# Rongjiehuang/FastDiff

Hardware: AMD Instinct MI355X
Metric: real-time factor (audio-sec/wall-sec), N=4 reverse steps, 80x864 mel (higher is better)
Workload: dtype f32 results; 2-piece fp16 operands (22 bit) on fp16 MFMA, fp32 accumulate; GEMM as Winograd F(2,3); exact-fp32 twin; 1 GPU; BASELINE configs[1]: LJSpeech shape, batch=8 x 80x864 mel per GPU, N=4, HIP kernels + hipGraph sampler; batch_per_gpu=8, frames=864, reverse_steps=4, graph=True, weights=random init seed 1234 (no checkpoint offline), world_size=1, gpus_visible=1, oversubscribed=False

## Files before the change

### fastdiff_amd/csrc/fd_kernels_lvc.hip

```cpp
#include "fd_kernels_common.h"

namespace fdk_fast {

template <int HOP, int DIL>
struct LvcCfg {
    static constexpr int WC = 64;
    static constexpr int W = 4 * WC;
    static constexpr int H = (DIL + 1 + 3) & ~3;
    static constexpr int XLD = W + 2 * H;
    static constexpr int YLD = W + 4;
};

#ifdef FD_LVC_TIMING
__device__ long long fd_dbg[64 * 4 * 8];
#define FD_STAMP(i) do { if (lane == 0 && blockIdx.y == FD_LVC_TIMING && blockIdx.x >= 100 && blockIdx.x < 164) \
        fd_dbg[((blockIdx.x - 100) * 4 + wave) * 8 + (i)] = (long long)__builtin_amdgcn_s_memtime(); } while (0)
#elif defined(FD_LVC_TIMELINE)
__device__ long long *fd_tl;
#define FD_STAMP_AT(i) do { if (threadIdx.x == 0) { long long *q_ = fd_tl + ((size_t)blockIdx.y * gridDim.x + blockIdx.x) * 10; \
        q_[i] = (long long)__builtin_amdgcn_s_memrealtime(); \
        if ((i) == 0) { q_[8] = __builtin_amdgcn_s_getreg(63492); q_[9] = __builtin_amdgcn_s_getreg(63508); } } } while (0)
#if defined(FD_TL_VARIANT)
#define FD_STAMP(i) do { if ((i) == 0 || (i) == 6 || (i) == 7) FD_STAMP_AT(i); else if ((i) == 1) FD_STAMP_AT(5); } while (0)
#define FD_STAMP_X(i) FD_STAMP_AT(i)
#else
#define FD_STAMP(i) FD_STAMP_AT(i)
#endif
#else
#define FD_STAMP(i)
#endif
#ifndef FD_STAMP_X
#define FD_STAMP_X(i)
#endif

__device__ __forceinline__ float gate(float a, float b)
{
    typedef float f2 __attribute__((ext_vector_type(2)));
    b = fmaxf(b, -15.0f);
    const f2 e = f2{a, b} * f2{-1.4426950408889634f, -2.8853900817779268f};
    const f2 uv = f2{__builtin_amdgcn_exp2f(e.x), __builtin_amdgcn_exp2f(e.y)};
    const f2 d = uv + 1.0f;
    return (1.0f - uv.y) * __builtin_amdgcn_rcpf(d.x * d.y);
}

template <int HOP, int DIL>
__global__ void __launch_bounds__(256, 2) k_lvc_layer(const float *__restrict__ xin, const float *__restrict__ skip,
                                                      float *__restrict__ xout, const float *__restrict__ kpack, int layer,
                                                      const float *__restrict__ wpack, const float *__restrict__ wref,
                                                      const float *__restrict__ cbias, int T, const int *__restrict__ run_if,
                                                      const int *__restrict__ lens)
{
    static_assert(HOP >= 64, "hop 8 has its own kernel (k_lvc_h8)");
    using Cfg = LvcCfg<HOP, DIL>;
    if (run_if && *run_if == 0) return;
    constexpr int WC = Cfg::WC, W = Cfg::W, H = Cfg::H, XLD = Cfg::XLD, YLD = Cfg::YLD, NT = WC / 32;
    constexpr int LT = (HOP == 256) ? 1 : 2;
    constexpr int LN = (HOP == 256) ? 4 : 2;
    constexpr bool PREACT = (HOP == 256);
    __shared__ __attribute__((aligned(16))) float xs[fd::C * XLD];
    __shared__ __attribute__((aligned(16))) float ys[fd::C * YLD];
    const int Ln = T * HOP;
    const int b = blockIdx.y, w0 = blockIdx.x * W;
    const int Tb = frames_of(lens, b, T), Lnb = Tb * HOP;
    if (w0 >= Lnb) return;
    const int tid = threadIdx.x, lane = tid & 63, wave = tid >> 6, l31 = lane & 31, hi = lane >> 5;
    const int cw = wave * WC;
    const bool wave_valid = (w0 + cw) < Lnb;
    const int mt0 = (HOP == 256) ? (wave & 1) : 0;
    const int lcw = (HOP == 256) ? 128 * (wave >> 1) : cw;
    FD_STAMP(0);

    float4 ka[LT][12];
    float4 bz[LT][4];
    if constexpr (HOP >= 64) {
        if (wave_valid) {
            const int f = (w0 + lcw) / HOP;
            const float *rec = kpack + ((int64_t)b * T + f) * fd::KREC;
            const float4 *kp4 = reinterpret_cast<const float4 *>(rec + layer * fd::KLAYER) + 2 * lane;
            const float4 *kb4 = reinterpret_cast<const float4 *>(rec + fd::KW + layer * 64);
#pragma unroll
            for (int m = 0; m < LT; ++m) {
#pragma unroll
                for (int i = 0; i < 12; ++i) ka[m][i] = kp4[((mt0 + m) * 6 + (i >> 1)) * 128 + (i & 1)];
#pragma unroll
                for (int j = 0; j < 4; ++j) bz[m][j] = kb4[(mt0 + m) * 8 + 2 * j + hi];
            }
        }
    }
    float4 wa[12];
#pragma unroll
    for (int i = 0; i < 12; ++i) wa[i] = reinterpret_cast<const float4 *>(wpack)[i * 64 + lane];
    float4 cb[4];
#pragma unroll
    for (int j = 0; j < 4; ++j) cb[j] = reinterpret_cast<const float4 *>(cbias)[2 * j + hi];
    {
        const float *xr = xin + (int64_t)b * fd::C * Ln, *sr = skip + (int64_t)b * fd::C * Ln;
        constexpr int NF4 = XLD / 4, TOTAL = fd::C * NF4, NK = (TOTAL + 255) / 256;
        constexpr int NB = (HOP == 64) ? 2 : 1, KB = (NK + NB - 1) / NB;
#pragma unroll
        for (int bt = 0; bt < NB; ++bt) {
            float4 xa[KB], sa[KB];
#pragma unroll
            for (int k = 0; k < KB; ++k) {
                const int idx = (bt * KB + k) * 256 + tid, ci = idx / NF4, c4 = idx - ci * NF4, g = w0 - H + 4 * c4;
                const bool ok = idx < TOTAL && g >= 0 && g < Lnb;
                xa[k] = ok ? *reinterpret_cast<const float4 *>(xr + (int64_t)ci * Ln + g) : make_float4(0.f, 0.f, 0.f, 0.f);
                sa[k] = ok ? *reinterpret_cast<const float4 *>(sr + (int64_t)ci * Ln + g) : make_float4(0.f, 0.f, 0.f, 0.f);
            }
            __builtin_amdgcn_sched_barrier(0);
#pragma unroll
            for (int k = 0; k < KB; ++k) {
                const int idx = (bt * KB + k) * 256 + tid, ci = idx / NF4, c4 = idx - ci * NF4;
                if (idx < TOTAL) {
                    const float4 r = make_float4(xa[k].x + sa[k].x, xa[k].y + sa[k].y, xa[k].z + sa[k].z, xa[k].w + sa[k].w);
                    if constexpr (PREACT) {
                        *reinterpret_cast<float4 *>(xs + ci * XLD + 4 * c4) =
                            make_float4(lrelu(r.x, 0.2f), lrelu(r.y, 0.2f), lrelu(r.z, 0.2f), lrelu(r.w, 0.2f));
                        if (c4 >= H / 4 && c4 < H / 4 + W / 4) *reinterpret_cast<float4 *>(ys + ci * YLD + 4 * c4 - H) = r;
                    } else {
                        *reinterpret_cast<float4 *>(xs + ci * XLD + 4 * c4) = r;
                    }
                }
            }
        }
    }
    const int hside = tid >> 7, ho = (tid & 127) >> 2, hq = tid & 3;
    __syncthreads();
    FD_STAMP(1);
    float resid[PREACT ? LN : 1][PREACT ? 8 * LT : 1];
    if constexpr (PREACT) {
#pragma unroll
        for (int nt = 0; nt < LN; ++nt)
#pragma unroll
            for (int m = 0; m < LT; ++m)
#pragma unroll
                for (int r = 0; r < 8; ++r)
                    resid[nt][m * 8 + r] = ys[(16 * (mt0 + m) + (r & 3) + 8 * (r >> 2) + 4 * hi) * YLD + lcw + nt * 32 + l31];
        __syncthreads();
    }

    if (wave_valid) {
        f32x16 acc[NT];
#pragma unroll
        for (int ct = 0; ct < NT; ++ct) {
#pragma unroll
            for (int r = 0; r < 16; ++r) acc[ct][r] = f4c(cb[r >> 2], r & 3);
            const int col = hi * XLD + H + cw + ct * 32 + l31;
            const int o[3] = {opaque(col - DIL), opaque(col), opaque(col + DIL)};
#pragma unroll
            for (int s = 0; s < 48; ++s) {
                const int tap = s >> 4, c2 = (2 * s) & 31;
                const float xv = xs[o[tap] + c2 * XLD];
                const float v = PREACT ? xv : lrelu(xv, 0.2f);
                acc[ct] = mfma32(f4c(wa[s >> 2], s & 3), v, acc[ct]);
                if (ct > 0 && s % 3 == 1) {
                    const int r = s / 3, cp = cw + (ct - 1) * 32 + l31;
                    ys[drow(r, hi) * YLD + cp + 1] = (w0 + cp) < Lnb ? lrelu(acc[ct - 1][r], 0.2f) : 0.0f;
                }
            }
        }
        {
            const int cp = cw + (NT - 1) * 32 + l31;
            const bool inside = (w0 + cp) < Lnb;
#pragma unroll
            for (int r = 0; r < 16; ++r) ys[drow(r, hi) * YLD + cp + 1] = inside ? lrelu(acc[NT - 1][r], 0.2f) : 0.0f;
        }
    } else {
#pragma unroll
        for (int ct = 0; ct < NT; ++ct)
#pragma unroll
            for (int r = 0; r < 16; ++r) ys[drow(r, hi) * YLD + cw + ct * 32 + l31 + 1] = 0.0f;
    }
    FD_STAMP(2);
    {
        float4 hwt[6];
#pragma unroll
        for (int j = 0; j < 6; ++j) hwt[j] = reinterpret_cast<const float4 *>(wref + (ho * fd::C + 8 * hq) * 3)[j];
        const float hbias = cbias[ho];
        const int c = hside ? W : -1, g = w0 + c;
        float accv = 0.0f;
        if (g >= 0 && g < Lnb) {
            const float wv[24] = {hwt[0].x, hwt[0].y, hwt[0].z, hwt[0].w, hwt[1].x, hwt[1].y, hwt[1].z, hwt[1].w,
                                  hwt[2].x, hwt[2].y, hwt[2].z, hwt[2].w, hwt[3].x, hwt[3].y, hwt[3].z, hwt[3].w,
                                  hwt[4].x, hwt[4].y, hwt[4].z, hwt[4].w, hwt[5].x, hwt[5].y, hwt[5].z, hwt[5].w};
#pragma unroll
            for (int j = 0; j < 8; ++j)
#pragma unroll
                for (int tap = 0; tap < 3; ++tap)
                {
                    const float xv = xs[(8 * hq + j) * XLD + H + c + (tap - 1) * DIL];
                    accv += wv[j * 3 + tap] * (PREACT ? xv : lrelu(xv, 0.2f));
                }
        }
        accv += __shfl_xor(accv, 1, 64);
        accv += __shfl_xor(accv, 2, 64);
        if (hq == 0) ys[ho * YLD + c + 1] = (g >= 0 && g < Lnb) ? lrelu(accv + hbias, 0.2f) : 0.0f;
    }
    FD_STAMP(3);
    __syncthreads();
    FD_STAMP(4);
    if (!wave_valid) return;

    const int64_t orow = (int64_t)b * fd::C * Ln;
    if constexpr (HOP >= 64) {
        float *xo = xout + orow + (int64_t)(4 * hi) * Ln + w0 + lcw + l31;
        const unsigned Lnu = (unsigned)Ln;
        f32x16 a[LN][LT];
        auto epilogue_row = [&](int nt, int m, int r) {
            const int chl = 16 * (mt0 + m) + (r & 3) + 8 * (r >> 2);
            float xr;
            if constexpr (PREACT) xr = resid[nt][m * 8 + r];
            else xr = xs[(chl + 4 * hi) * XLD + H + lcw + nt * 32 + l31];
            xo[(unsigned)chl * Lnu + (unsigned)(nt * 32)] = xr + gate(a[nt][m][r], a[nt][m][r + 8]);
        };
        constexpr int EPI = 8 * LT, GAP = 48 / EPI;
#pragma unroll
        for (int nt = 0; nt < LN; ++nt) {
#pragma unroll
            for (int m = 0; m < LT; ++m)
#pragma unroll
                for (int r = 0; r < 16; ++r) a[nt][m][r] = f4c(bz[m][r >> 2], r & 3);
            const int yc = hi * 8 * YLD + lcw + nt * 32 + l31;
            const int yo[3] = {opaque(yc), opaque(yc + 1), opaque(yc + 2)};
#pragma unroll
            for (int s = 0; s < 48; ++s) {
                const int tap = s >> 4, c2 = 16 * ((s >> 3) & 1) + (s & 7);
                const float v = ys[yo[tap] + c2 * YLD];
#pragma unroll
                for (int m = 0; m < LT; ++m) a[nt][m] = mfma32(f4c(ka[m][s >> 2], s & 3), v, a[nt][m]);
                if (nt > 0 && s % GAP == GAP / 2) {
                    const int e = s / GAP;
                    epilogue_row(nt - 1, e / 8, e % 8);
                }
            }
            if (nt == 0) FD_STAMP(5);
        }
        FD_STAMP(6);
#pragma unroll
        for (int e = 0; e < EPI; ++e) epilogue_row(LN - 1, e / 8, e % 8);
        FD_STAMP(7);
    }
}

template <int HOP, int DIL, bool FINAL, int UP = 0>
__global__ void __launch_bounds__(256, 2) k_lvc_h2(const float *__restrict__ xin, const float *__restrict__ skip, float *__restrict__ xout,
                                                   const float *__restrict__ kpack, int layer, const float4 *__restrict__ wpack16,
                                                   const float *__restrict__ wref, const float *__restrict__ cbias,
                                                   int *__restrict__ range_flag, int T, const int *__restrict__ lens,
                                                   float *__restrict__ eps_acc, const float4 *__restrict__ ffuse,
                                                   const float4 *__restrict__ up_pack16, const float *__restrict__ up_bias,
                                                   int *__restrict__ up_flag)
{
    static_assert(!FINAL || HOP == 256, "the fused final conv relies on whole-tile utterance lengths");
    static_assert(UP == 0 || (DIL == 1 && (UP == 4 || UP == 8)), "the fused up-sampler belongs to the first layer of a block");
    constexpr int W = 256, WC = 64, H = (DIL + 1 + 3) & ~3, XC = W + 2 * H, YC = W + 2;
    constexpr int UPPAD = UP ? UP : 1, UPN = UP ? (W + 2 * UPPAD) / UPPAD : 0, UPROWS = UPN + 2;
    __shared__ __attribute__((aligned(16))) char xp_img[UP ? UPROWS * 128 : 16];
    __shared__ float hsk[UP ? fd::C * 2 * H : 1];
    constexpr int LT = (HOP == 256) ? 1 : 2;
    constexpr int LN = (HOP == 256) ? 4 : 2;
    static_assert(2 * H <= 64, "one halo column per lane");
    __shared__ __attribute__((aligned(16))) char xs[XC * 128];
    __shared__ __attribute__((aligned(16))) char ys[YC * 128];
    static_assert(YC * 128 >= fd::C * W * 4, "parking area");
    const int Ln = T * HOP;
    const int ntile = (T * HOP + W - 1) / W, tile = lvc_tile_of_workgroup();
    const int b = blockIdx.y, w0 = tile * W;
    const int Lnb = frames_of(lens, b, T) * HOP;
    if (tile >= ntile || w0 >= Lnb || skip_after_previous_overflow(range_flag)) return;
    const int tid = threadIdx.x, lane = tid & 63, wave = tid >> 6, l31 = lane & 31, hi = lane >> 5;
    const int cw = wave * WC;
    const bool wave_valid = (w0 + cw) < Lnb;
    const int mt0 = (HOP == 256) ? (wave & 1) : 0;
    const int lcw = (HOP == 256) ? 128 * (wave >> 1) : cw;
    float mx = 0.0f;
    FD_STAMP(0);

    float4 ka[LT][12];
    float4 bz[LT][4];
    auto load_kernel = [&](int m) {
        if (HOP == 256 || wave_valid) {
            const int f = (w0 + lcw) / HOP;
            const float *rec = kpack + ((int64_t)b * T + f) * fd::KREC;
            const float4 *kp4 = reinterpret_cast<const float4 *>(rec + layer * fd::KLAYER) + 2 * lane;
            const float4 *kb4 = reinterpret_cast<const float4 *>(rec + fd::KW + layer * 64);
#pragma unroll
            for (int i = 0; i < 12; ++i) ka[m][i] = lvc_ld<4>(kp4 + ((mt0 + m) * 6 + (i >> 1)) * 128 + (i & 1));
#pragma unroll
            for (int j = 0; j < 4; ++j) bz[m][j] = kb4[(mt0 + m) * 8 + 2 * j + hi];
        }
    };
    __shared__ float4 ffs[FINAL ? 64 : 1];
    if constexpr (FINAL) {
        if (tid < 64) ffs[tid] = ffuse[tid];
    }
#ifndef FD_LVC_LATE_KERNEL
    if constexpr (HOP == 256) load_kernel(0);
#endif
    float4 wa[2][6];
    float4 cb[4];
    float hbias;
    auto load_conv_weights = [&]() {
#pragma unroll
        for (int p = 0; p < 2; ++p)
#pragma unroll
            for (int kg = 0; kg < 6; ++kg) wa[p][kg] = wpack16[(p * 6 + kg) * 64 + lane];
#pragma unroll
        for (int j = 0; j < 4; ++j) cb[j] = reinterpret_cast<const float4 *>(cbias)[2 * j + hi];
        hbias = cbias[l31];
    };
    if constexpr (UP == 0) load_conv_weights();
#ifdef FD_LVC_PAD_LOADS
    {
        float4 pad_[FD_LVC_PAD_LOADS];
#pragma unroll
        for (int i_ = 0; i_ < FD_LVC_PAD_LOADS; ++i_) pad_[i_] = wpack16[(i_ % 12) * 64 + lane];
#pragma unroll
        for (int i_ = 0; i_ < FD_LVC_PAD_LOADS; ++i_) mx = fmaxf(mx, fminf(pad_[i_].x, 0.0f) * 1e-30f);
    }
#endif

    {
        const float *xr = xin + ((int64_t)b * fd::C + wave * 8) * Ln, *sr = skip + ((int64_t)b * fd::C + wave * 8) * Ln;
        const int g = w0 + 4 * lane;
        const bool ok = g < Lnb;
        const int hc = lane, hg = (hc < H) ? w0 - H + hc : w0 + W + hc - H;
        const bool hok = hc < 2 * H && hg >= 0 && hg < Lnb;
        float4 xa[8], sa[8];
        float hx[8], hs[8];
#pragma unroll
        for (int c = 0; c < 8; ++c) {
#ifdef FD_LVC_PROBE_NOLOADX
            const float pv_ = __int_as_float(0x3c000000 | (lane << 8) | (c << 4));
            if constexpr (UP == 0) xa[c] = make_float4(pv_, -pv_, pv_ * 0.5f, pv_ * 0.25f);
            sa[c] = make_float4(pv_ * 0.125f, pv_, -pv_, pv_ * 2.0f);
#else
            if constexpr (UP == 0) xa[c] = ok ? lvc_ld<1>(reinterpret_cast<const float4 *>(xr + (int64_t)c * Ln + g)) : make_float4(0.f, 0.f, 0.f, 0.f);
            sa[c] = ok ? lvc_ld<8>(reinterpret_cast<const float4 *>(sr + (int64_t)c * Ln + g)) : make_float4(0.f, 0.f, 0.f, 0.f);
#endif
        }
#pragma unroll
        for (int c = 0; c < 8; ++c) {
#ifdef FD_LVC_PROBE_NOLOADX
            if constexpr (UP == 0) hx[c] = __int_as_float(0x3b000000 | (lane << 8) | (c << 4));
            hs[c] = hok ? 0.03125f : 0.0f;
#else
            if constexpr (UP == 0) hx[c] = hok ? xr[(int64_t)c * Ln + hg] : 0.0f;
            hs[c] = hok ? sr[(int64_t)c * Ln + hg] : 0.0f;
#endif
        }
#ifdef FD_LVC_PROBE_UP_NOCONVT
        if constexpr (UP > 0) {
            load_conv_weights();
#pragma unroll
            for (int c = 0; c < 8; ++c) {
                const float pv_ = __int_as_float(0x3c000000 | (lane << 8) | (c << 4));
                xa[c] = make_float4(pv_, -pv_, pv_ * 0.5f, pv_ * 0.25f);
                hx[c] = pv_ * 0.125f;
            }
            (void)xp_img; (void)hsk; (void)up_pack16; (void)up_bias;
        }
#else
        if constexpr (UP > 0) {
            constexpr int R = UP, NT = (UPN + 31) / 32, PHW = R / 4;
            const int Lq = Ln / R, Lqb = Lnb / R, q0 = w0 / R;
            {
                constexpr int NU = 4 * UPROWS, NK = (NU + 255) / 256;
                float v[NK][8];
#pragma unroll
                for (int k = 0; k < NK; ++k) {
                    const int u = k * 256 + tid, cg = u / UPROWS, jj = u - cg * UPROWS, j = q0 - 2 + jj;
                    const bool okp = u < NU && j >= 0 && j < Lqb;
#pragma unroll
                    for (int c = 0; c < 8; ++c) v[k][c] = okp ? xin[((int64_t)b * fd::C + cg * 8 + c) * Lq + j] : 0.0f;
                }
#pragma unroll
                for (int k = 0; k < NK; ++k) {
                    const int u = k * 256 + tid, cg = u / UPROWS, jj = u - cg * UPROWS;
                    if (u < NU) {
#pragma unroll
                        for (int c = 0; c < 8; ++c) { mx = fmaxf(mx, fabsf(v[k][c])); v[k][c] = lrelu(v[k][c], 0.2f); }
                        float4 ph, pl;
                        split8(v[k], ph, pl);
                        *reinterpret_cast<float4 *>(xp_img + h2_off(jj, cg)) = ph;
                        *reinterpret_cast<float4 *>(xp_img + h2_off(jj, 4 + cg)) = pl;
                    }
                }
            }
            float4 ub[4];
#pragma unroll
            for (int j = 0; j < 4; ++j) ub[j] = reinterpret_cast<const float4 *>(up_bias)[2 * j + hi];
            float4 wun[2][4];
#pragma unroll
            for (int p = 0; p < 2; ++p)
#pragma unroll
                for (int kg = 0; kg < 4; ++kg) wun[p][kg] = up_pack16[(((wave * PHW) * 2 + p) * 4 + kg) * 64 + lane];
            __syncthreads();
            FD_STAMP_X(1);
            float *park = reinterpret_cast<float *>(ys);
#pragma unroll
            for (int pw = 0; pw < PHW; ++pw) {
                const int ph = wave * PHW + pw;
                float4 wu[2][4];
#pragma unroll
                for (int p = 0; p < 2; ++p)
#pragma unroll
                    for (int kg = 0; kg < 4; ++kg) wu[p][kg] = wun[p][kg];
                if (pw + 1 < PHW) {
#pragma unroll
                    for (int p = 0; p < 2; ++p)
#pragma unroll
                        for (int kg = 0; kg < 4; ++kg) wun[p][kg] = up_pack16[(((ph + 1) * 2 + p) * 4 + kg) * 64 + lane];
                }
                const int offA = (ph < R / 2) ? 0 : 1, offB = offA - 1;
#pragma unroll
                for (int t = 0; t < NT; ++t) {
                    const int ql = 32 * t + l31, qc = min(ql, UPN - 1);
                    f32x16 ah, al;
#pragma unroll
                    for (int r = 0; r < 16; ++r) { ah[r] = f4c(ub[r >> 2], r & 3); al[r] = 0.0f; }
#pragma unroll
                    for (int kg = 0; kg < 4; ++kg) {
                        const int row = qc + 1 + ((kg >> 1) ? offB : offA), c2 = kg & 1;
                        const float4 b1 = *reinterpret_cast<const float4 *>(xp_img + h2_off(row, c2 * 2 + hi));
                        const float4 b2 = *reinterpret_cast<const float4 *>(xp_img + h2_off(row, 4 + c2 * 2 + hi));
                        ah = mfma_f16(wu[0][kg], b1, ah);
                        al = mfma_f16(wu[0][kg], b2, al);
                        al = mfma_f16(wu[1][kg], b1, al);
                    }
                    const int col = R * ql + ph - UPPAD;
                    if (ql < UPN && col >= -H && col < W + H) {
                        const int gc = w0 + col;
                        const bool inb = gc >= 0 && gc < Lnb;
                        const int pcol = ph * (W / R) + ((ql - 1) ^ ((R == 8) ? 16 * (ph >> 2) : 0));
                        float *dst = (col >= 0 && col < W) ? park + pcol : hsk + (col < 0 ? col + H : col - W + H);
                        const int cs = (col >= 0 && col < W) ? W : 2 * H;
#pragma unroll
                        for (int r = 0; r < 16; ++r)
                            dst[(8 * (r >> 2) + 4 * hi + (r & 3)) * cs] = inb ? fmaf(al[r], GX_INV_SCALE, ah[r]) : 0.0f;
                    }
                }
            }
            FD_STAMP_X(2);
            __syncthreads();
            FD_STAMP_X(3);
            load_conv_weights();
            {
                const float *pk = reinterpret_cast<const float *>(ys) + wave * 8 * W +
                                  (R == 4 ? lane : (4 * (lane & 1)) * (W / R) + ((lane >> 1) ^ (16 * (lane & 1))));
#pragma unroll
                for (int c = 0; c < 8; ++c)
                    xa[c] = make_float4(pk[c * W], pk[c * W + (W / R)], pk[c * W + 2 * (W / R)], pk[c * W + 3 * (W / R)]);
            }
#pragma unroll
            for (int c = 0; c < 8; ++c) hx[c] = hc < 2 * H ? hsk[(wave * 8 + c) * (2 * H) + hc] : 0.0f;
            FD_STAMP_X(4);
        }
#endif
#ifdef FD_LVC_LATE_KERNEL
        __builtin_amdgcn_sched_barrier(0);
        if constexpr (HOP == 256 && UP == 0) load_kernel(0);
#endif
        __builtin_amdgcn_sched_barrier(0);
#pragma unroll
        for (int c = 0; c < 8; ++c) {
            xa[c] = make_float4(xa[c].x + sa[c].x, xa[c].y + sa[c].y, xa[c].z + sa[c].z, xa[c].w + sa[c].w);
            mx = amax4(mx, xa[c]);
            *reinterpret_cast<float4 *>(ys + ((wave * 8 + c) * W + 4 * lane) * 4) = xa[c];
        }
#pragma unroll
        for (int j = 0; j < 4; ++j) {
            float v[8];
#pragma unroll
            for (int c = 0; c < 8; ++c) v[c] = lrelu(f4c(xa[c], j), 0.2f);
            float4 ph, pl;
            split8(v, ph, pl);
            const int row = H + 4 * lane + j;
            *reinterpret_cast<float4 *>(xs + h2_off(row, wave)) = ph;
            *reinterpret_cast<float4 *>(xs + h2_off(row, 4 + wave)) = pl;
        }
        if (hc < 2 * H) {
            float v[8];
#pragma unroll
            for (int c = 0; c < 8; ++c) {
                const float t = hx[c] + hs[c];
                mx = fmaxf(mx, fabsf(t));
                v[c] = lrelu(t, 0.2f);
            }
            float4 ph, pl;
            split8(v, ph, pl);
            const int row = (hc < H) ? hc : W + hc;
            *reinterpret_cast<float4 *>(xs + h2_off(row, wave)) = ph;
            *reinterpret_cast<float4 *>(xs + h2_off(row, 4 + wave)) = pl;
        }
    }
    if constexpr (HOP != 256) load_kernel(0);
    __syncthreads();
    FD_STAMP(1);
    float resid[LN][8 * LT];
    {
#pragma unroll
        for (int nt = 0; nt < LN; ++nt)
#pragma unroll
            for (int m = 0; m < LT; ++m)
#pragma unroll
                for (int r = 0; r < 8; ++r)
                    resid[nt][m * 8 + r] =
                        reinterpret_cast<const float *>(ys)[(16 * (mt0 + m) + (r & 3) + 8 * (r >> 2) + 4 * hi) * W + lcw + nt * 32 + l31];
        __syncthreads();
    }
    FD_STAMP(2);

    if (wave_valid) {
        int xo_[3][2][2];
#pragma unroll
        for (int tap = 0; tap < 3; ++tap) {
            const int row = H + cw + l31 + (tap - 1) * DIL;
#pragma unroll
            for (int p = 0; p < 2; ++p)
#pragma unroll
                for (int c2 = 0; c2 < 2; ++c2) xo_[tap][p][c2] = h2_off(row, p * 4 + c2 * 2 + hi);
        }
#pragma unroll
        for (int ct = 0; ct < 2; ++ct) {
            f32x16 ah, al;
#pragma unroll
            for (int r = 0; r < 16; ++r) { ah[r] = f4c(cb[r >> 2], r & 3); al[r] = 0.0f; }
#pragma unroll
            for (int kg = 0; kg < 6; ++kg) {
                const float4 b1 = *reinterpret_cast<const float4 *>(xs + xo_[kg >> 1][0][kg & 1] + ct * 32 * 128);
                const float4 b2 = *reinterpret_cast<const float4 *>(xs + xo_[kg >> 1][1][kg & 1] + ct * 32 * 128);
                ah = mfma_f16(wa[0][kg], b1, ah);
                al = mfma_f16(wa[0][kg], b2, al);
                al = mfma_f16(wa[1][kg], b1, al);
            }
            const int cp = cw + ct * 32 + l31, yrow = cp + 1;
            const bool inside = (w0 + cp) < Lnb;
#pragma unroll
            for (int j = 0; j < 4; ++j) {
                float v[4];
#pragma unroll
                for (int i = 0; i < 4; ++i) {
                    v[i] = inside ? lrelu(fmaf(al[4 * j + i], GX_INV_SCALE, ah[4 * j + i]), 0.2f) : 0.0f;
                    mx = fmaxf(mx, fabsf(v[i]));
                }
                uint2 ph, pl;
                split2(v[0], v[1], ph.x, pl.x);
                split2(v[2], v[3], ph.y, pl.y);
                *reinterpret_cast<uint2 *>(ys + h2_off(yrow, j) + 8 * hi) = ph;
                *reinterpret_cast<uint2 *>(ys + h2_off(yrow, 4 + j) + 8 * hi) = pl;
            }
        }
    } else {
#pragma unroll
        for (int s8 = 0; s8 < 8; ++s8) *reinterpret_cast<float4 *>(ys + (cw + 1 + lane) * 128 + s8 * 16) = make_float4(0.f, 0.f, 0.f, 0.f);
    }
    if constexpr (HOP != 256) load_kernel(1);
    FD_STAMP(3);
    if (wave < 2) {
        const int c = wave ? W : -1, g = w0 + c;
        const bool ok = g >= 0 && g < Lnb;
        float a1 = 0.0f, a2 = 0.0f;
        if (ok) {
#pragma unroll
            for (int kg = 0; kg < 6; ++kg) halo_dot(xs, H + c + ((kg >> 1) - 1) * DIL, (kg & 1) * 2 + hi, wa[0][kg], wa[1][kg], a1, a2);
        }
        float accv = fmaf(a2, GX_INV_SCALE, a1);
        accv += __shfl_xor(accv, 32, 64);
        if (hi == 0) {
            const float v = ok ? lrelu(accv + hbias, 0.2f) : 0.0f;
            mx = fmaxf(mx, fabsf(v));
            const _Float16 v1 = (_Float16)v, v2 = (_Float16)((v - (float)v1) * GX_SCALE);
            const int yrow = c + 1;
            *reinterpret_cast<_Float16 *>(ys + h2_off(yrow, l31 >> 3) + (l31 & 7) * 2) = v1;
            *reinterpret_cast<_Float16 *>(ys + h2_off(yrow, 4 + (l31 >> 3)) + (l31 & 7) * 2) = v2;
        }
    }
    FD_STAMP(4);
    __syncthreads();
    FD_STAMP(5);
    if (wave_valid) {
        float4 kh[LT][6], kl[LT][6];
#pragma unroll
        for (int m = 0; m < LT; ++m)
#pragma unroll
            for (int kg = 0; kg < 6; ++kg) {
                const float4 &a0 = ka[m][2 * kg], &a1 = ka[m][2 * kg + 1];
                mx = amax4(amax4(mx, a0), a1);
                const float v[8] = {a0.x, a0.y, a0.z, a0.w, a1.x, a1.y, a1.z, a1.w};
                split8(v, kh[m][kg], kl[m][kg]);
            }
        int yo_[3][2][2];
#pragma unroll
        for (int tap = 0; tap < 3; ++tap) {
            const int row = lcw + l31 + tap;
#pragma unroll
            for (int p = 0; p < 2; ++p)
#pragma unroll
                for (int c2 = 0; c2 < 2; ++c2) yo_[tap][p][c2] = h2_off(row, p * 4 + c2 * 2 + hi);
        }
        const int64_t ooff = (int64_t)b * fd::C * Ln + (int64_t)(4 * hi) * Ln + w0 + lcw + l31;
        float *xo = xout + ooff;
        FD_STAMP(6);
#ifdef FD_LVC_PAD_VALU
        {
            float pad_ = mx;
#pragma unroll
            for (int i_ = 0; i_ < FD_LVC_PAD_VALU; ++i_) asm volatile("v_fma_f32 %0, %0, %0, %0" : "+v"(pad_));
            mx = fminf(mx, pad_ * 0.0f + mx);
        }
#endif
        const unsigned Lnu = (unsigned)Ln;
#pragma unroll
        for (int nt = 0; nt < LN; ++nt) {
#pragma unroll
            for (int m = 0; m < LT; ++m) {
                f32x16 ah, al;
#pragma unroll
                for (int r = 0; r < 16; ++r) { ah[r] = f4c(bz[m][r >> 2], r & 3); al[r] = 0.0f; }
#pragma unroll
                for (int kg = 0; kg < 6; ++kg) {
                    const float4 b1 = *reinterpret_cast<const float4 *>(ys + yo_[kg >> 1][0][kg & 1] + nt * 32 * 128);
                    const float4 b2 = *reinterpret_cast<const float4 *>(ys + yo_[kg >> 1][1][kg & 1] + nt * 32 * 128);
                    ah = mfma_f16(kh[m][kg], b1, ah);
                    al = mfma_f16(kh[m][kg], b2, al);
                    al = mfma_f16(kl[m][kg], b1, al);
                }
#pragma unroll
                for (int r = 0; r < 8; ++r) {
                    const int chl = 16 * (mt0 + m) + (r & 3) + 8 * (r >> 2);
                    const float zs = fmaf(al[r], GX_INV_SCALE, ah[r]), zt = fmaf(al[r + 8], GX_INV_SCALE, ah[r + 8]);
                    if constexpr (FINAL) resid[nt][m * 8 + r] += gate(zs, zt);
#ifdef FD_LVC_PROBE_NOSTORE
                    else { const float keep_ = resid[nt][m * 8 + r] + gate(zs, zt); asm volatile("" :: "v"(keep_)); (void)xo; (void)Lnu; (void)chl; }
#else
                    else lvc_st<2>(xo + ((unsigned)chl * Lnu + (unsigned)(nt * 32)), resid[nt][m * 8 + r] + gate(zs, zt));
#endif
                }
            }
        }
    }
#ifdef FD_LVC_PROBE_FINAL_NOFOLD
    if constexpr (FINAL) {
#pragma unroll
        for (int nt = 0; nt < LN; ++nt)
#pragma unroll
            for (int r = 0; r < 8; ++r) asm volatile("" :: "v"(resid[nt][r]));
        (void)eps_acc; (void)ffs;
    }
#else
    if constexpr (FINAL) {
        FD_STAMP_X(1);
        float *pb = reinterpret_cast<float *>(xs);
        {
            const int part = 2 * mt0 + hi;
            float fw[8][8];
#pragma unroll
            for (int r = 0; r < 8; ++r) {
                const float4 lo4 = ffs[(part * 8 + r) * 2], hi4 = ffs[(part * 8 + r) * 2 + 1];
                fw[r][0] = lo4.x; fw[r][1] = lo4.y; fw[r][2] = lo4.z; fw[r][3] = lo4.w; fw[r][4] = hi4.x; fw[r][5] = hi4.y; fw[r][6] = hi4.z;
            }
#pragma unroll
            for (int nt = 0; nt < LN; ++nt)
#pragma unroll
                for (int k = 0; k < 7; ++k) {
                    float pk = 0.0f;
#pragma unroll
                    for (int r = 0; r < 8; ++r) pk = fmaf(fw[r][k], resid[nt][r], pk);
                    pb[(part * 7 + k) * W + lcw + nt * 32 + l31] = pk;
                }
        }
        FD_STAMP_X(2);
        __syncthreads();
        FD_STAMP_X(3);
        auto column_sum = [&](int t) {
            float e = 0.0f;
#pragma unroll
            for (int k = 0; k < 7; ++k) {
                const int col = t + k - 3;
                if (col >= 0 && col < W) {
#pragma unroll
                    for (int part = 0; part < 4; ++part) e += pb[(part * 7 + k) * W + col];
                }
            }
            return e;
        };
        float *ea = eps_acc + (int64_t)b * Ln + w0;
        const float e = column_sum(tid);
        if (tid >= 3 && tid < W - 3) ea[tid] = e;
        else atomicAdd(ea + tid, e);
        if (tid >= 64 && tid < 70) {
            const int j = tid - 64, t = j < 3 ? j - 3 : W + j - 3;
            if (w0 + t >= 0 && w0 + t < Lnb) atomicAdd(ea + t, column_sum(t));
        }
        FD_STAMP_X(4);
    }
#endif
    if (!(mx < GX_LIMIT)) {
        atomicOr(range_flag, 1);
        if constexpr (UP > 0) atomicOr(up_flag, 1);
    }
    FD_STAMP(7);
}
template <int DIL>
__global__ void __launch_bounds__(256, 2) k_lvc_h8(const float *__restrict__ xin, const float *__restrict__ skip, float *__restrict__ xout,
                                                   const float *__restrict__ kpack, int layer, const float *__restrict__ wref,
                                                   const float *__restrict__ cbias, int T, const int *__restrict__ lens,
                                                   const int *__restrict__ run_if)
{
    constexpr int HOP = 8, W = 32, H = (DIL + 1 + 3) & ~3, XLD = W + 2 * H, YLD = 12;
    if (run_if && *run_if == 0) return;
    __shared__ __attribute__((aligned(16))) float xs[fd::C * XLD];
    __shared__ __attribute__((aligned(16))) float xr[fd::C * W];
    __shared__ __attribute__((aligned(16))) float ys[4][fd::C * YLD];
    __shared__ float wl[fd::C * 3 * fd::C];
    const int Ln = T * HOP;
    const int b = blockIdx.y, w0 = blockIdx.x * W;
    const int Tb = frames_of(lens, b, T), Lnb = Tb * HOP;
    if (w0 >= Lnb) return;
    const int tid = threadIdx.x, lane = tid & 63, wave = tid >> 6, l31 = lane & 31, hi = lane >> 5;
    const int f = w0 / HOP + wave;
    const bool frame_valid = f < Tb;
    float4 ke[12], ko[12];
    float bzv = 0.0f;
    if (frame_valid) {
        const float *rec = kpack + ((int64_t)b * T + f) * fd::KREC;
        const float4 *kp4 = reinterpret_cast<const float4 *>(rec + layer * fd::KLAYER) + (hi * 6 * 64 + l31) * 2;
#pragma unroll
        for (int i = 0; i < 12; ++i) { ke[i] = kp4[(i >> 1) * 128 + (i & 1)]; ko[i] = kp4[(i >> 1) * 128 + 64 + (i & 1)]; }
        bzv = rec[fd::KW + layer * 64 + lane];
    }
    float wst[12];
#pragma unroll
    for (int k = 0; k < 12; ++k) { const int idx = k * 256 + tid; wst[k] = wref[(idx & 31) * (fd::C * 3) + (idx >> 5)]; }
    const float cbv = cbias[l31];
    {
        const float *xp = xin + (int64_t)b * fd::C * Ln, *sp = skip + (int64_t)b * fd::C * Ln;
        constexpr int NF4 = XLD / 4, TOTAL = fd::C * NF4, NK = (TOTAL + 255) / 256;
        float4 xa[NK], sa[NK];
#pragma unroll
        for (int k = 0; k < NK; ++k) {
            const int idx = k * 256 + tid, ci = idx / NF4, c4 = idx - ci * NF4, g = w0 - H + 4 * c4;
            const bool ok = idx < TOTAL && g >= 0 && g < Lnb;
            xa[k] = ok ? *reinterpret_cast<const float4 *>(xp + (int64_t)ci * Ln + g) : make_float4(0.f, 0.f, 0.f, 0.f);
            sa[k] = ok ? *reinterpret_cast<const float4 *>(sp + (int64_t)ci * Ln + g) : make_float4(0.f, 0.f, 0.f, 0.f);
        }
#pragma unroll
        for (int k = 0; k < NK; ++k) {
            const int idx = k * 256 + tid, ci = idx / NF4, c4 = idx - ci * NF4;
            if (idx < TOTAL) {
                const float4 r = make_float4(xa[k].x + sa[k].x, xa[k].y + sa[k].y, xa[k].z + sa[k].z, xa[k].w + sa[k].w);
                *reinterpret_cast<float4 *>(xs + ci * XLD + 4 * c4) = make_float4(lrelu(r.x, 0.2f), lrelu(r.y, 0.2f), lrelu(r.z, 0.2f), lrelu(r.w, 0.2f));
                if (c4 >= H / 4 && c4 < H / 4 + W / 4) *reinterpret_cast<float4 *>(xr + ci * W + 4 * c4 - H) = r;
            }
        }
    }
#pragma unroll
    for (int k = 0; k < 12; ++k) wl[k * 256 + tid] = wst[k];
    __syncthreads();
    if (!frame_valid) return;
    {
        float acc[5] = {cbv, cbv, cbv, cbv, cbv};
        const float *xb = xs + H + 8 * wave - 1 + 5 * hi;
#pragma unroll 2
        for (int in = 0; in < fd::C; ++in)
#pragma unroll
            for (int k = 0; k < 3; ++k) {
                const float wv = wl[(in * 3 + k) * fd::C + l31];
                const float *xq = xb + in * XLD + (k - 1) * DIL;
#pragma unroll
                for (int c = 0; c < 5; ++c) acc[c] = fmaf(wv, xq[c], acc[c]);
            }
#pragma unroll
        for (int c = 0; c < 5; ++c) {
            const int g = w0 + 8 * wave - 1 + 5 * hi + c;
            ys[wave][l31 * YLD + 5 * hi + c] = (g >= 0 && g < Lnb) ? lrelu(acc[c], 0.2f) : 0.0f;
        }
    }
    __builtin_amdgcn_fence(__ATOMIC_RELEASE, "wavefront");
    __builtin_amdgcn_wave_barrier();
    float z[8];
#pragma unroll
    for (int c = 0; c < 8; ++c) z[c] = bzv;
#pragma unroll
    for (int in = 0; in < fd::C; ++in) {
        const float *yr = ys[wave] + in * YLD;
        const float4 y0 = *reinterpret_cast<const float4 *>(yr);
        const float4 y1 = *reinterpret_cast<const float4 *>(yr + 4);
        const float2 y2 = *reinterpret_cast<const float2 *>(yr + 8);
        const float yv[10] = {y0.x, y0.y, y0.z, y0.w, y1.x, y1.y, y1.z, y1.w, y2.x, y2.y};
#pragma unroll
        for (int tap = 0; tap < 3; ++tap) {
            const int kk = tap * 32 + in, kg = kk >> 4, e = kk & 7;
            const float kv = (kk & 8) ? f4c(ko[2 * kg + (e >> 2)], e & 3) : f4c(ke[2 * kg + (e >> 2)], e & 3);
#pragma unroll
            for (int c = 0; c < 8; ++c) z[c] = fmaf(kv, yv[c + tap], z[c]);
        }
    }
#pragma unroll
    for (int c = 0; c < 8; ++c) {
        const float zt = __shfl_down(z[c], 16, 64);
        z[c] = gate(z[c], zt);
    }
    if ((lane & 16) == 0) {
        const int ch = 16 * hi + (lane & 15), c0 = 8 * wave;
        float *dst = xout + ((int64_t)b * fd::C + ch) * Ln + w0 + c0;
        const float *rr = xr + ch * W + c0;
        *reinterpret_cast<float4 *>(dst) = make_float4(rr[0] + z[0], rr[1] + z[1], rr[2] + z[2], rr[3] + z[3]);
        *reinterpret_cast<float4 *>(dst + 4) = make_float4(rr[4] + z[4], rr[5] + z[5], rr[6] + z[6], rr[7] + z[7]);
    }
}
// ... 286 lines not shown
```

Before: 9993 x real-time.

## Fuse up-sampler epilogue directly into residual and split conv input writes

In the fused up-sampler path, the transposed-conv MFMA epilogue now adds the skip input, which is prefetched into registers, computes leaky-ReLU, and writes the fp16 hi/lo split straight into the conv input tile and a swizzled float4 residual slot. This removes the parking pass through shared memory, a __syncthreads, the re-read into registers and the separate halo buffer. The residual reload for this path becomes swizzled float4 loads. It costs more registers for the prefetched skip values (PHW*NT*16 floats) and uses clamped, uncoalesced per-column global loads.

```diff
diff --git a/fastdiff_amd/csrc/fd_kernels_lvc.hip b/fastdiff_amd/csrc/fd_kernels_lvc.hip
--- a/fastdiff_amd/csrc/fd_kernels_lvc.hip
+++ b/fastdiff_amd/csrc/fd_kernels_lvc.hip
@@ -242,6 +242,13 @@
     }
 }
 
+template <int R>
+__device__ __forceinline__ int up_resid_slot(int hi, int col)
+{
+    const int ph = col & (R - 1), q = col / R;
+    return (hi * R + ph) * (256 / R) + (q ^ ((R == 8 ? 2 : 4) * ph));
+}
+
 template <int HOP, int DIL, bool FINAL, int UP = 0>
 __global__ void __launch_bounds__(256, 2) k_lvc_h2(const float *__restrict__ xin, const float *__restrict__ skip, float *__restrict__ xout,
                                                    const float *__restrict__ kpack, int layer, const float4 *__restrict__ wpack16,
@@ -256,7 +263,6 @@
     constexpr int W = 256, WC = 64, H = (DIL + 1 + 3) & ~3, XC = W + 2 * H, YC = W + 2;
     constexpr int UPPAD = UP ? UP : 1, UPN = UP ? (W + 2 * UPPAD) / UPPAD : 0, UPROWS = UPN + 2;
     __shared__ __attribute__((aligned(16))) char xp_img[UP ? UPROWS * 128 : 16];
-    __shared__ float hsk[UP ? fd::C * 2 * H : 1];
     constexpr int LT = (HOP == 256) ? 1 : 2;
     constexpr int LN = (HOP == 256) ? 4 : 2;
     static_assert(2 * H <= 64, "one halo column per lane");
@@ -320,7 +326,118 @@
     }
 #endif
 
-    {
+#ifdef FD_LVC_PROBE_UP_NOCONVT
+    constexpr bool UPD = false;
+#else
+    constexpr bool UPD = UP > 0;
+#endif
+    if constexpr (UPD) {
+        constexpr int R = UP, NT = (UPN + 31) / 32, PHW = R / 4;
+        const int Lq = Ln / R, Lqb = Lnb / R, q0 = w0 / R;
+        float sk[PHW][NT][16];
+        {
+            const float *sb = skip + (int64_t)b * fd::C * Ln;
+            const unsigned Lnu = (unsigned)Ln;
+#pragma unroll
+            for (int pw = 0; pw < PHW; ++pw)
+#pragma unroll
+                for (int t = 0; t < NT; ++t) {
+                    const int gc = w0 + R * (32 * t + l31) + wave * PHW + pw - UPPAD;
+                    const unsigned u = (unsigned)(4 * hi) * Lnu + (unsigned)min(max(gc, 0), Lnb - 1);
+#pragma unroll
+                    for (int r = 0; r < 16; ++r) sk[pw][t][r] = sb[(unsigned)(8 * (r >> 2) + (r & 3)) * Lnu + u];
+                }
+        }
+        {
+            constexpr int NU = 4 * UPROWS, NK = (NU + 255) / 256;
+            float v[NK][8];
+#pragma unroll
+            for (int k = 0; k < NK; ++k) {
+                const int u = k * 256 + tid, cg = u / UPROWS, jj = u - cg * UPROWS, j = q0 - 2 + jj;
+                const bool okp = u < NU && j >= 0 && j < Lqb;
+#pragma unroll
+                for (int c = 0; c < 8; ++c) v[k][c] = okp ? xin[((int64_t)b * fd::C + cg * 8 + c) * Lq + j] : 0.0f;
+            }
+#pragma unroll
+            for (int k = 0; k < NK; ++k) {
+                const int u = k * 256 + tid, cg = u / UPROWS, jj = u - cg * UPROWS;
+                if (u < NU) {
+#pragma unroll
+                    for (int c = 0; c < 8; ++c) { mx = fmaxf(mx, fabsf(v[k][c])); v[k][c] = lrelu(v[k][c], 0.2f); }
+                    float4 ph, pl;
+                    split8(v[k], ph, pl);
+                    *reinterpret_cast<float4 *>(xp_img + h2_off(jj, cg)) = ph;
+                    *reinterpret_cast<float4 *>(xp_img + h2_off(jj, 4 + cg)) = pl;
+                }
+            }
+        }
+        float4 ub[4];
+#pragma unroll
+        for (int j = 0; j < 4; ++j) ub[j] = reinterpret_cast<const float4 *>(up_bias)[2 * j + hi];
+        float4 wun[2][4];
+#pragma unroll
+        for (int p = 0; p < 2; ++p)
+#pragma unroll
+            for (int kg = 0; kg < 4; ++kg) wun[p][kg] = up_pack16[(((wave * PHW) * 2 + p) * 4 + kg) * 64 + lane];
+        __syncthreads();
+        FD_STAMP_X(1);
+#pragma unroll
+        for (int pw = 0; pw < PHW; ++pw) {
+            const int ph = wave * PHW + pw;
+            float4 wu[2][4];
+#pragma unroll
+            for (int p = 0; p < 2; ++p)
+#pragma unroll
+                for (int kg = 0; kg < 4; ++kg) wu[p][kg] = wun[p][kg];
+            if (pw + 1 < PHW) {
+#pragma unroll
+                for (int p = 0; p < 2; ++p)
+#pragma unroll
+                    for (int kg = 0; kg < 4; ++kg) wun[p][kg] = up_pack16[(((ph + 1) * 2 + p) * 4 + kg) * 64 + lane];
+            }
+            const int offA = (ph < R / 2) ? 0 : 1, offB = offA - 1;
+#pragma unroll
+            for (int t = 0; t < NT; ++t) {
+                const int ql = 32 * t + l31, qc = min(ql, UPN - 1);
+                f32x16 ah, al;
+#pragma unroll
+                for (int r = 0; r < 16; ++r) { ah[r] = f4c(ub[r >> 2], r & 3); al[r] = 0.0f; }
+#pragma unroll
+                for (int kg = 0; kg < 4; ++kg) {
+                    const int row = qc + 1 + ((kg >> 1) ? offB : offA), c2 = kg & 1;
+                    const float4 b1 = *reinterpret_cast<const float4 *>(xp_img + h2_off(row, c2 * 2 + hi));
+                    const float4 b2 = *reinterpret_cast<const float4 *>(xp_img + h2_off(row, 4 + c2 * 2 + hi));
+                    ah = mfma_f16(wu[0][kg], b1, ah);
+                    al = mfma_f16(wu[0][kg], b2, al);
+                    al = mfma_f16(wu[1][kg], b1, al);
+                }
+                const int col = R * ql + ph - UPPAD;
+                if (ql < UPN && col >= -H && col < W + H) {
+                    const int gc = w0 + col;
+                    const bool inb = gc >= 0 && gc < Lnb, centre = col >= 0 && col < W;
+                    float4 *rs = reinterpret_cast<float4 *>(ys) + up_resid_slot<R>(hi, centre ? col : 0);
+                    const int xrow = H + col;
+#pragma unroll
+                    for (int j = 0; j < 4; ++j) {
+                        float v[4];
+#pragma unroll
+                        for (int i = 0; i < 4; ++i) {
+                            v[i] = inb ? fmaf(al[4 * j + i], GX_INV_SCALE, ah[4 * j + i]) + sk[pw][t][4 * j + i] : 0.0f;
+                            mx = fmaxf(mx, fabsf(v[i]));
+                        }
+                        if (centre) rs[j * (2 * W)] = make_float4(v[0], v[1], v[2], v[3]);
+                        uint2 ph2, pl2;
+                        split2(lrelu(v[0], 0.2f), lrelu(v[1], 0.2f), ph2.x, pl2.x);
+                        split2(lrelu(v[2], 0.2f), lrelu(v[3], 0.2f), ph2.y, pl2.y);
+                        *reinterpret_cast<uint2 *>(xs + h2_off(xrow, j) + 8 * hi) = ph2;
+                        *reinterpret_cast<uint2 *>(xs + h2_off(xrow, 4 + j) + 8 * hi) = pl2;
+                    }
+                }
+            }
+        }
+        FD_STAMP_X(2);
+        load_conv_weights();
+    } else {
         const float *xr = xin + ((int64_t)b * fd::C + wave * 8) * Ln, *sr = skip + ((int64_t)b * fd::C + wave * 8) * Ln;
         const int g = w0 + 4 * lane;
         const bool ok = g < Lnb;
@@ -358,103 +475,7 @@
                 xa[c] = make_float4(pv_, -pv_, pv_ * 0.5f, pv_ * 0.25f);
                 hx[c] = pv_ * 0.125f;
             }
-            (void)xp_img; (void)hsk; (void)up_pack16; (void)up_bias;
-        }
-#else
-        if constexpr (UP > 0) {
-            constexpr int R = UP, NT = (UPN + 31) / 32, PHW = R / 4;
-            const int Lq = Ln / R, Lqb = Lnb / R, q0 = w0 / R;
-            {
-                constexpr int NU = 4 * UPROWS, NK = (NU + 255) / 256;
-                float v[NK][8];
-#pragma unroll
-                for (int k = 0; k < NK; ++k) {
-                    const int u = k * 256 + tid, cg = u / UPROWS, jj = u - cg * UPROWS, j = q0 - 2 + jj;
-                    const bool okp = u < NU && j >= 0 && j < Lqb;
-#pragma unroll
-                    for (int c = 0; c < 8; ++c) v[k][c] = okp ? xin[((int64_t)b * fd::C + cg * 8 + c) * Lq + j] : 0.0f;
-                }
-#pragma unroll
-                for (int k = 0; k < NK; ++k) {
-                    const int u = k * 256 + tid, cg = u / UPROWS, jj = u - cg * UPROWS;
-                    if (u < NU) {
-#pragma unroll
-                        for (int c = 0; c < 8; ++c) { mx = fmaxf(mx, fabsf(v[k][c])); v[k][c] = lrelu(v[k][c], 0.2f); }
-                        float4 ph, pl;
-                        split8(v[k], ph, pl);
-                        *reinterpret_cast<float4 *>(xp_img + h2_off(jj, cg)) = ph;
-                        *reinterpret_cast<float4 *>(xp_img + h2_off(jj, 4 + cg)) = pl;
-                    }
-                }
-            }
-            float4 ub[4];
-#pragma unroll
-            for (int j = 0; j < 4; ++j) ub[j] = reinterpret_cast<const float4 *>(up_bias)[2 * j + hi];
-            float4 wun[2][4];
-#pragma unroll
-            for (int p = 0; p < 2; ++p)
-#pragma unroll
-                for (int kg = 0; kg < 4; ++kg) wun[p][kg] = up_pack16[(((wave * PHW) * 2 + p) * 4 + kg) * 64 + lane];
-            __syncthreads();
-            FD_STAMP_X(1);
-            float *park = reinterpret_cast<float *>(ys);
-#pragma unroll
-            for (int pw = 0; pw < PHW; ++pw) {
-                const int ph = wave * PHW + pw;
-                float4 wu[2][4];
-#pragma unroll
-                for (int p = 0; p < 2; ++p)
-#pragma unroll
-                    for (int kg = 0; kg < 4; ++kg) wu[p][kg] = wun[p][kg];
-                if (pw + 1 < PHW) {
-#pragma unroll
-                    for (int p = 0; p < 2; ++p)
-#pragma unroll
-                        for (int kg = 0; kg < 4; ++kg) wun[p][kg] = up_pack16[(((ph + 1) * 2 + p) * 4 + kg) * 64 + lane];
-                }
-                const int offA = (ph < R / 2) ? 0 : 1, offB = offA - 1;
-#pragma unroll
-                for (int t = 0; t < NT; ++t) {
-                    const int ql = 32 * t + l31, qc = min(ql, UPN - 1);
-                    f32x16 ah, al;
-#pragma unroll
-                    for (int r = 0; r < 16; ++r) { ah[r] = f4c(ub[r >> 2], r & 3); al[r] = 0.0f; }
-#pragma unroll
-                    for (int kg = 0; kg < 4; ++kg) {
-                        const int row = qc + 1 + ((kg >> 1) ? offB : offA), c2 = kg & 1;
-                        const float4 b1 = *reinterpret_cast<const float4 *>(xp_img + h2_off(row, c2 * 2 + hi));
-                        const float4 b2 = *reinterpret_cast<const float4 *>(xp_img + h2_off(row, 4 + c2 * 2 + hi));
-                        ah = mfma_f16(wu[0][kg], b1, ah);
-                        al = mfma_f16(wu[0][kg], b2, al);
-                        al = mfma_f16(wu[1][kg], b1, al);
-                    }
-                    const int col = R * ql + ph - UPPAD;
-                    if (ql < UPN && col >= -H && col < W + H) {
-                        const int gc = w0 + col;
-                        const bool inb = gc >= 0 && gc < Lnb;
-                        const int pcol = ph * (W / R) + ((ql - 1) ^ ((R == 8) ? 16 * (ph >> 2) : 0));
-                        float *dst = (col >= 0 && col < W) ? park + pcol : hsk + (col < 0 ? col + H : col - W + H);
-                        const int cs = (col >= 0 && col < W) ? W : 2 * H;
-#pragma unroll
-                        for (int r = 0; r < 16; ++r)
-                            dst[(8 * (r >> 2) + 4 * hi + (r & 3)) * cs] = inb ? fmaf(al[r], GX_INV_SCALE, ah[r]) : 0.0f;
-                    }
-                }
-            }
-            FD_STAMP_X(2);
-            __syncthreads();
-            FD_STAMP_X(3);
-            load_conv_weights();
-            {
-                const float *pk = reinterpret_cast<const float *>(ys) + wave * 8 * W +
-                                  (R == 4 ? lane : (4 * (lane & 1)) * (W / R) + ((lane >> 1) ^ (16 * (lane & 1))));
-#pragma unroll
-                for (int c = 0; c < 8; ++c)
-                    xa[c] = make_float4(pk[c * W], pk[c * W + (W / R)], pk[c * W + 2 * (W / R)], pk[c * W + 3 * (W / R)]);
-            }
-#pragma unroll
-            for (int c = 0; c < 8; ++c) hx[c] = hc < 2 * H ? hsk[(wave * 8 + c) * (2 * H) + hc] : 0.0f;
-            FD_STAMP_X(4);
+            (void)xp_img; (void)up_pack16; (void)up_bias;
         }
 #endif
 #ifdef FD_LVC_LATE_KERNEL
@@ -503,10 +524,19 @@
         for (int nt = 0; nt < LN; ++nt)
 #pragma unroll
             for (int m = 0; m < LT; ++m)
-#pragma unroll
-                for (int r = 0; r < 8; ++r)
-                    resid[nt][m * 8 + r] =
-                        reinterpret_cast<const float *>(ys)[(16 * (mt0 + m) + (r & 3) + 8 * (r >> 2) + 4 * hi) * W + lcw + nt * 32 + l31];
+                if constexpr (UPD) {
+#pragma unroll
+                    for (int jj = 0; jj < 2; ++jj) {
+                        const float4 q4 = reinterpret_cast<const float4 *>(ys)[(2 * (mt0 + m) + jj) * (2 * W) + up_resid_slot<UPPAD>(hi, lcw + nt * 32 + l31)];
+                        resid[nt][m * 8 + 4 * jj] = q4.x; resid[nt][m * 8 + 4 * jj + 1] = q4.y;
+                        resid[nt][m * 8 + 4 * jj + 2] = q4.z; resid[nt][m * 8 + 4 * jj + 3] = q4.w;
+                    }
+                } else {
+#pragma unroll
+                    for (int r = 0; r < 8; ++r)
+                        resid[nt][m * 8 + r] =
+                            reinterpret_cast<const float *>(ys)[(16 * (mt0 + m) + (r & 3) + 8 * (r >> 2) + 4 * hi) * W + lcw + nt * 32 + l31];
+                }
         __syncthreads();
     }
     FD_STAMP(2);
```

New measurement: 9715 x real-time. 0.972x the previous value.
